# nico-bohlinger/RL-X

Measured on AMD Instinct MI355X. Metric: env-steps/sec (whole node) PPO 4096 envs at 1/2/4/8 MI355X, higher is better.
Workload: dtype f32

## Files before the change

rl-x_amd/csrc/common.h:

```cpp
#pragma once
#include <hip/hip_runtime.h>
#include <hip/hip_ext.h>
#include <stdint.h>
#include <cstring>
#include <cmath>
#include <string>
#include <vector>
#include <functional>
#include "../../include/rlx_hip.h"

namespace rlx {

void set_error(const std::string& msg);

#define RLX_HIP_TRY(expr)                                                                      \
  do {                                                                                         \
    hipError_t e_ = (expr);                                                                    \
    if (e_ != hipSuccess) {                                                                    \
      ::rlx::set_error(std::string(#expr) + " failed: " + hipGetErrorString(e_) + " (" __FILE__ \
                       ":" + std::to_string(__LINE__) + ")");                                  \
      return RLX_EHIP;                                                                         \
    }                                                                                          \
  } while (0)

#define RLX_REQUIRE(cond, code, msg)                 \
  do {                                               \
    if (!(cond)) {                                   \
      ::rlx::set_error(std::string(msg));            \
      return (code);                                 \
    }                                                \
  } while (0)

#define RLX_LAUNCH_CHECK()                           \
  RLX_HIP_TRY(hipGetLastError())

constexpr int WAVE = 64;

struct Scratch {
  void* ptr = nullptr;
  size_t bytes = 0;
};

enum ScratchSlot {
  SL_SORT_KEYS_A = 0, SL_SORT_KEYS_B, SL_SORT_VALS_B, SL_SORT_TMP, SL_PERM,
  SL_MB_X, SL_MB_XC, SL_MB_AUX, SL_STATS,
  SL_ACT_P0, SL_ACT_P1, SL_ACT_P2, SL_ACT_C0, SL_ACT_C1, SL_ACT_C2,
  SL_DACT_0, SL_DACT_1, SL_LN_P, SL_LN_C,
  SL_PARTIAL, SL_HEAD_PART, SL_NORM, SL_NORM2, SL_FWD_A, SL_FWD_B, SL_KEYS, SL_GRAD_P, SL_GRAD_C, SL_MEAN, SL_VALUE, SL_RO_NETS, SL_SAC, SL_LSTM, SL_LSTM_IDX, SL_STAGE, SL_OPT_A, SL_OPT_B, SL_STATS_ALL, SL_ZEROS, SL_STAT_PART, SL_LIDX, SL_COUNTS, SL_DIST_STATS, SL_OVERFLOW, SL_SCHED, SL_NV_ROWS, SL_WFRAG, SL_WFRAG_RO, SL_XMAX, SL_MB_GROUP_X, SL_MB_GROUP_AUX, SL_DZ0, SL_WFRAG_SAC, SL_ROW_REC,
  SL_COUNT
};

enum ProfKernel { PK_GEMM_FWD = 0, PK_GEMM_DX, PK_GEMM_DW, PK_DX_L1BWD,
                  PK_L1FWD, PK_HEAD_LOSS, PK_REDUCE,
                  PK_L12FWD,
                  PK_TAIL,
                  PK_FWD2H,
                  PK_COUNT };
constexpr int PROF_ENGINE_HBM = 2;
struct ProfRec {
  int kid, row;
  double flops, bytes;
  hipEvent_t e0, e1;
};
struct ProfRow {
  int kid, engine;
  int64_t M;
  int N, K;
  int64_t launches, timed;
  double ms, flops, bytes;
};
struct Twin { const void* p[4] = {nullptr, nullptr, nullptr, nullptr}; };

}

struct AttrOnce {
  uint64_t mask = 0;
  static int dev() { int d = 0; (void)hipGetDevice(&d); return d & 63; }
  bool done() const { return (mask >> dev()) & 1; }
  void mark() { mask |= 1ull << dev(); }
};

struct rlx_ctx {
  int device = 0;
  rlx::Scratch slots[3][rlx::SL_COUNT];
  int bank = 0;
  int opt_flip = 0;
  hipStream_t side = nullptr;
  hipEvent_t ev_fork = nullptr, ev_join = nullptr;
  hipEvent_t ev_rows[2] = {nullptr, nullptr};
  hipEvent_t ev_cdone[2] = {nullptr, nullptr};
  const float* dbg_sac_eps[2] = {nullptr, nullptr};
  bool l1fwd_mfma = true;
  bool pipeline_updates = true;
  bool pf_valid = false;
  uint32_t pf_key_in[2] = {0, 0}, pf_key_out[2] = {0, 0};
  int pf_E = 0, pf_scheme = 0;
  int64_t pf_B = 0;
  hipEvent_t pf_done = nullptr;
  hipEvent_t ev_perm_free = nullptr;
  bool perm_free_recorded = false;
  bool two_streams = true;
  const uint32_t* l1_xmax = nullptr;
  const uint32_t* xmax_slot[2] = {nullptr, nullptr};
  int lf_idle_cus = 0;
  bool dw_recompute = false;
  float* l12_stats = nullptr;
  bool l12_ran = false;
  int l1_stats_handover = 1;
  int l1_wrap_refill = 1;
  int64_t dx_l1bwd_wrap_launches = 0;
  int l12_prefetch = 1;
  int64_t l12fwd_pf_launches = 0;
  float* l1_hand_req = nullptr;
  const float* l1_hand[2] = {nullptr, nullptr};
  bool dw_merge = true;
  void* dbg_stamps = nullptr;
  bool fwd2h = true;
  int gather_group_rows = 524288;
  bool gather_records = true;
  bool l12_fused = true;
  int ppo_tail = -1;
  int tail32_waves = 8;
  int ln_row_once = 1;
  int ppo_twin = -1;
  bool fused_recurrent_act = true;
  int num_cus = 256;
  void* defer = nullptr;
  bool prof_on = false;
  int prof_sample = 1;
  hipEvent_t prof_ref = nullptr;
  double prof_union_ms = 0.0;
  std::vector<rlx::ProfRec> prof_recs;
  std::vector<rlx::ProfRow> prof_rows;
  std::vector<hipEvent_t> prof_pool;
  bool gemm_bx = true;
  float bx_gscale = 1.f;
  bool adam_emit = true;
  bool bx_keep[3] = {false, false, false};
  struct RoImages { bool valid = false; const float* params[2] = {nullptr, nullptr}; const void* img[2][3] = {}; int nt[2][3] = {}; } ro_img;
  int bx_force_mi = 0;
  int bx_debug = 0;
  struct BxImage { const float* W; int trans, K, N; const void* img; };
  BxImage bx_img[3][32];
  int bx_n[3] = {0, 0, 0};
  bool disable_l1fused = false;
  std::vector<char> ro_nets_shadow;
  int rank = 0, world = 1;
  void* comm = nullptr;
  hipStream_t comm_stream = nullptr;
  hipEvent_t comm_ev[32] = {};
  int comm_ev_pos = 0;
  rlx_allreduce_fn ar_hook = nullptr;
  void* ar_hook_user = nullptr;
  int ro_exit = 0;
  int64_t bx_window_fallbacks = 0;
  int64_t ar_calls = 0;
  hipStream_t sac_st[2] = {nullptr, nullptr};
  hipEvent_t sac_ev[6] = {nullptr, nullptr, nullptr, nullptr, nullptr, nullptr};
  struct SacImages {
    bool valid = false; const float *pp = nullptr, *qp = nullptr, *qt = nullptr; rlx_mlp_desc pd{}, qd{}; int64_t np = 0, nq2 = 0;
    void written(const float* p, int64_t n) {
      if (!valid) return;
      auto hit = [&](const float* b, int64_t m) { return b && p < b + m && b < p + n; };
      if (hit(pp, np) || hit(qp, nq2) || hit(qt, nq2)) valid = false;
    }
  } sac_img;
  const void* sac_img_arena = nullptr;
  int sac_twin = 1;
  float* sched_host[4] = {nullptr, nullptr, nullptr, nullptr};
  hipEvent_t sched_ev[4] = {nullptr, nullptr, nullptr, nullptr};
  size_t sched_cap = 0;
  int sched_pos = 0;
  int espo_chunk = 2;
  int32_t* espo_host = nullptr;
  hipEvent_t espo_ev[3] = {nullptr, nullptr, nullptr};
  bool pf_dist = false;
  int pf_T = 0, pf_nl = 0, pf_ng = 0, pf_off = 0, pf_mb = 0;
};

namespace rlx {

struct ProfScope {
  rlx_ctx* ctx;
  hipStream_t st;
  int idx = -1;
  ProfScope(rlx_ctx* c, int kid, double flops, hipStream_t s, double bytes = 0.0, int64_t M = 0, int N = 0, int K = 0,
            int engine = 0);
  hipEvent_t ev0() const;
  hipEvent_t ev1() const;
};
#define RLX_PLAUNCH(KERNEL, GRID, BLOCK, LDS, ST, ...)                                                              \
  do {                                                                                                            \
    if (prof.idx >= 0) hipExtLaunchKernelGGL(KERNEL, GRID, BLOCK, LDS, ST, prof.ev0(), prof.ev1(), 0, __VA_ARGS__); \
    else hipLaunchKernelGGL(KERNEL, GRID, BLOCK, LDS, ST, __VA_ARGS__);                                           \
  } while (0)

inline double gemm_bytes(double M, double N, double K, int c_rw = 0) { return 4.0 * (M * K + K * N + M * N * (1 + c_rw)); }

const float* zeros_f32(rlx_ctx* ctx, size_t n);
int ctx_side_stream(rlx_ctx* ctx);
int ctx_sac_streams(rlx_ctx* ctx);
__host__ __device__ __forceinline__ float x_pow2_inv(float m) {
  union { float f; uint32_t u; } c;
  c.f = m;
  const int e = (int)((c.u >> 23) & 0xffu);
  if (e == 0 || e == 0xff) return 1.f;
  int se = 254 - e;
// ... 298 lines not shown
```

rl-x_amd/csrc/core.hip:

```cpp
#include "common.h"
#include <algorithm>
#include <cstdio>
#include <cstdlib>
#include <utility>

namespace rlx {

static thread_local std::string g_last_error;

void set_error(const std::string& msg) { g_last_error = msg; }

void* scratch(rlx_ctx* ctx, ScratchSlot s, size_t bytes) {
  Scratch& sl = ctx->slots[ctx->bank][s];
  if (sl.bytes >= bytes && sl.ptr) return sl.ptr;
  if (sl.ptr) {
    if (hipDeviceSynchronize() != hipSuccess) { set_error("hipDeviceSynchronize failed in scratch()"); return nullptr; }
    (void)hipFree(sl.ptr);
    sl.ptr = nullptr;
    sl.bytes = 0;
  }
  size_t want = ((bytes > (size_t(1) << 20) ? bytes + bytes / 8 : bytes) + 255) & ~size_t(255);
  void* p = nullptr;
  hipError_t e = hipMalloc(&p, want);
  if (e != hipSuccess) {
// ... 145 lines not shown
      flops_out[r.kid] += r.flops;
      bytes_out[r.kid] += r.bytes;
      count_out[r.kid] += 1;
      rlx::ProfRow& q = ctx->prof_rows[r.row];
      q.timed += 1;
      q.ms += ms;
      q.flops += r.flops;
      q.bytes += r.bytes;
      if (q.engine != rlx::PROF_ENGINE_HBM && ctx->prof_ref && hipEventElapsedTime(&t0, ctx->prof_ref, r.e0) == hipSuccess)
        iv.emplace_back(t0, t0 + ms);
    }
    ctx->prof_pool.push_back(r.e0);
    ctx->prof_pool.push_back(r.e1);
  }
  ctx->prof_recs.clear();
  std::sort(iv.begin(), iv.end());
  double uni = 0.0;
  float cs = 0.f, ce = -1.f;
  for (auto& p : iv) {
    if (ce < 0.f || p.first > ce) { if (ce >= 0.f) uni += ce - cs; cs = p.first; ce = p.second; }
    else if (p.second > ce) ce = p.second;
  }
  if (ce >= 0.f) uni += ce - cs;
  ctx->prof_union_ms = uni;
  return RLX_OK;
}

int rlx_prof_rows(rlx_ctx* ctx, rlx_prof_row* rows, int capacity, int* n_out) {
  RLX_REQUIRE(ctx && n_out && (rows || capacity == 0), RLX_EINVAL, "rlx_prof_rows: NULL pointer");
  const int n = (int)ctx->prof_rows.size();
  *n_out = n;
  for (int i = 0; i < n && i < capacity; ++i) {
    const rlx::ProfRow& q = ctx->prof_rows[i];
    rows[i] = rlx_prof_row{q.kid, q.engine, q.N, q.K, q.M, q.launches, q.timed, q.ms, q.flops, q.bytes};
  }
  return RLX_OK;
}

int rlx_prof_union_ms(rlx_ctx* ctx, double* out) {
  RLX_REQUIRE(ctx && out, RLX_EINVAL, "rlx_prof_union_ms: NULL pointer");
  *out = ctx->prof_union_ms;
  return RLX_OK;
}

int rlx_dbg_set_option(rlx_ctx* ctx, const char* name, int value) {
  RLX_REQUIRE(ctx && name, RLX_EINVAL, "rlx_dbg_set_option: NULL");
  if (std::string(name) == "sac_twin") { ctx->sac_twin = value; return RLX_OK; }
  if (std::string(name) == "disable_l1fused") { ctx->disable_l1fused = value != 0; return RLX_OK; }
  if (std::string(name) == "l1fwd_mfma") { ctx->l1fwd_mfma = value != 0; return RLX_OK; }
  if (std::string(name) == "pipeline_updates") { ctx->pipeline_updates = value != 0; return RLX_OK; }
  if (std::string(name) == "two_streams") { ctx->two_streams = value != 0; return RLX_OK; }
  if (std::string(name) == "ppo_twin") { ctx->ppo_twin = value; return RLX_OK; }
  if (std::string(name) == "ro_exit") { ctx->ro_exit = value; return RLX_OK; }
  if (std::string(name) == "lf_idle_cus") { ctx->lf_idle_cus = value < 0 ? 0 : value; return RLX_OK; }
  if (std::string(name) == "dw_recompute") { ctx->dw_recompute = value != 0; return RLX_OK; }
  if (std::string(name) == "dw_merge") { ctx->dw_merge = value != 0; return RLX_OK; }
  if (std::string(name) == "fwd2h") { ctx->fwd2h = value != 0; return RLX_OK; }
  if (std::string(name) == "l12_fused") { ctx->l12_fused = value != 0; return RLX_OK; }
  if (std::string(name) == "gather_group_rows") { ctx->gather_group_rows = value; return RLX_OK; }
  if (std::string(name) == "gather_records") { ctx->gather_records = value != 0; return RLX_OK; }
  if (std::string(name) == "ppo_tail") { ctx->ppo_tail = value < 0 ? -1 : (value > 2 ? 2 : value); return RLX_OK; }
  if (std::string(name) == "tail32_waves") {
    RLX_REQUIRE(value == 4 || value == 8, RLX_EINVAL, "rlx_dbg_set_option: tail32_waves is 4 or 8");
    ctx->tail32_waves = value;
    return RLX_OK;
  }
  if (std::string(name) == "ln_row_once") {
    RLX_REQUIRE(value == 0 || value == 1, RLX_EINVAL, "rlx_dbg_set_option: ln_row_once is 0 or 1");
    ctx->ln_row_once = value;
    return RLX_OK;
  }
  if (std::string(name) == "l1_stats_handover") {
    RLX_REQUIRE(value == 0 || value == 1, RLX_EINVAL, "rlx_dbg_set_option: l1_stats_handover is 0 or 1");
    ctx->l1_stats_handover = value;
    return RLX_OK;
  }
  if (std::string(name) == "l1_wrap_refill") {
    RLX_REQUIRE(value == 0 || value == 1, RLX_EINVAL, "rlx_dbg_set_option: l1_wrap_refill is 0 or 1");
    ctx->l1_wrap_refill = value;
    return RLX_OK;
  }
  if (std::string(name) == "l12_prefetch") {
    RLX_REQUIRE(value == 0 || value == 1, RLX_EINVAL, "rlx_dbg_set_option: l12_prefetch is 0 or 1");
    ctx->l12_prefetch = value;
    return RLX_OK;
  }
  if (std::string(name) == "bx_force_mi") { ctx->bx_force_mi = value; return RLX_OK; }
  if (std::string(name) == "adam_emit") { ctx->adam_emit = value != 0; return RLX_OK; }
  if (std::string(name) == "bx_debug") { ctx->bx_debug = value; return RLX_OK; }
  if (std::string(name) == "bx_gscale_log2") { ctx->bx_gscale = ldexpf(1.f, value < 0 ? 0 : (value > 40 ? 40 : value)); return RLX_OK; }
  if (std::string(name) == "gemm_bx") { ctx->gemm_bx = value != 0; return RLX_OK; }
  if (std::string(name) == "prof_sample") { ctx->prof_sample = value < 1 ? 1 : value; return RLX_OK; }
  if (std::string(name) == "espo_chunk") { ctx->espo_chunk = value < 1 ? 1 : value; return RLX_OK; }
  if (std::string(name) == "fused_recurrent_act") { ctx->fused_recurrent_act = value != 0; return RLX_OK; }
  RLX_REQUIRE(false, RLX_EINVAL, "rlx_dbg_set_option: unknown option");
}

int rlx_dbg_get_counter(rlx_ctx* ctx, const char* name, int64_t* out) {
  RLX_REQUIRE(ctx && name && out, RLX_EINVAL, "rlx_dbg_get_counter: NULL");
  int bank = 0, slot = 0;
  if (sscanf(name, "scratch_ptr:%d:%d", &bank, &slot) == 2 && bank >= 0 && bank < 3 && slot >= 0 && slot < rlx::SL_COUNT) {
    *out = (int64_t)reinterpret_cast<uintptr_t>(ctx->slots[bank][slot].ptr);
    return RLX_OK;
  }
  if (sscanf(name, "scratch_bytes:%d:%d", &bank, &slot) == 2 && bank >= 0 && bank < 3 && slot >= 0 && slot < rlx::SL_COUNT) {
    *out = (int64_t)ctx->slots[bank][slot].bytes;
    return RLX_OK;
  }
  if (std::string(name) == "allreduce_calls") { *out = ctx->ar_calls; return RLX_OK; }
  if (std::string(name) == "dx_l1bwd_wrap_launches") { *out = ctx->dx_l1bwd_wrap_launches; return RLX_OK; }
  if (std::string(name) == "l12fwd_pf_launches") { *out = ctx->l12fwd_pf_launches; return RLX_OK; }
  if (std::string(name) == "bx_window_fallbacks") { *out = ctx->bx_window_fallbacks; return RLX_OK; }
  if (std::string(name) == "gemm_bx") { *out = ctx->gemm_bx ? 1 : 0; return RLX_OK; }
  RLX_REQUIRE(false, RLX_EINVAL, "rlx_dbg_get_counter: unknown counter");
}

int rlx_version(void) { return 200; }

const char* rlx_last_error(void) { return rlx::g_last_error.c_str(); }

int rlx_ctx_create(int device, rlx_ctx** out) {
  RLX_REQUIRE(out != nullptr, RLX_EINVAL, "rlx_ctx_create: out is NULL");
  int count = 0;
  RLX_HIP_TRY(hipGetDeviceCount(&count));
  RLX_REQUIRE(device >= 0 && device < count, RLX_EINVAL, "rlx_ctx_create: no such HIP device");
  RLX_HIP_TRY(hipSetDevice(device));
  hipDeviceProp_t prop;
  RLX_HIP_TRY(hipGetDeviceProperties(&prop, device));
  rlx_ctx* c = new rlx_ctx();
  c->device = device;
  c->num_cus = prop.multiProcessorCount;
  if (const char* e = getenv("RLX_GEMM_BX")) c->gemm_bx = atoi(e) != 0;
  if (const char* e = getenv("RLX_BX_DEBUG")) c->bx_debug = atoi(e);
  *out = c;
  return RLX_OK;
}

int rlx_dist_release(rlx_ctx* ctx);

int rlx_ctx_destroy(rlx_ctx* ctx) {
  if (!ctx) return RLX_OK;
  (void)hipSetDevice(ctx->device);
  (void)hipDeviceSynchronize();
  (void)rlx_dist_release(ctx);
  for (int i = 0; i < 2; ++i)
    if (ctx->sac_st[i]) (void)hipStreamDestroy(ctx->sac_st[i]);
  for (int i = 0; i < 6; ++i)
    if (ctx->sac_ev[i]) (void)hipEventDestroy(ctx->sac_ev[i]);
  for (int i = 0; i < 4; ++i) {
    if (ctx->sched_host[i]) (void)hipHostFree(ctx->sched_host[i]);
    if (ctx->sched_ev[i]) (void)hipEventDestroy(ctx->sched_ev[i]);
  }
  if (ctx->espo_host) (void)hipHostFree(ctx->espo_host);
  for (int i = 0; i < 3; ++i)
    if (ctx->espo_ev[i]) (void)hipEventDestroy(ctx->espo_ev[i]);
  for (int b = 0; b < 3; ++b)
    for (int i = 0; i < rlx::SL_COUNT; ++i)
      if (ctx->slots[b][i].ptr) (void)hipFree(ctx->slots[b][i].ptr);
  if (ctx->ev_fork) (void)hipEventDestroy(ctx->ev_fork);
  if (ctx->ev_join) (void)hipEventDestroy(ctx->ev_join);
  for (int p = 0; p < 2; ++p) {
    if (ctx->ev_rows[p]) (void)hipEventDestroy(ctx->ev_rows[p]);
    if (ctx->ev_cdone[p]) (void)hipEventDestroy(ctx->ev_cdone[p]);
  }
// ... 17 lines not shown
```

rl-x_amd/csrc/rollout.hip:

```cpp
#include "env_device.h"
#include "gemm.h"
#include "mlp.h"
#include "gemm_bx.h"
#include "ppo_internal.h"

namespace rlx {

constexpr int RO_ROWS = 32;
constexpr int RO_THREADS = 256;
constexpr int RO_MAXH = 512;
constexpr int RO_MAXN = 256;
constexpr int RO_A0 = RO_ROWS * (RO_MAXH + 1);
constexpr int RO_A1 = RO_ROWS * (RO_MAXN + 1);
constexpr int RO_BS = G_BK * (RO_MAXN + 4);
constexpr int RO_MISC = 1024 + 64;
constexpr int RO_LDS_FLOATS = RO_A0 + RO_A1 + RO_BS + RO_MISC;
constexpr float RO_LOG_2PI = 1.8378770664093453f;

#define RO_ACT_SWITCH(ACTV, ...)                                                                                      \
  if ((ACTV) == RLX_ACT_ELU) { auto actf = [](float v_) { return act_fwd_t<RLX_ACT_ELU>(v_); }; __VA_ARGS__ }          \
  else if ((ACTV) == RLX_ACT_TANH) { auto actf = [](float v_) { return act_fwd_t<RLX_ACT_TANH>(v_); }; __VA_ARGS__ }   \
  else { const int act_rt_ = (ACTV); auto actf = [act_rt_](float v_) { return act_fwd(v_, act_rt_); }; __VA_ARGS__ }

struct RolloutNet {
// ... 572 lines not shown
          a.env.final_obs[o] = ox[q];
          if (2 * p + 1 < O) a.env.final_obs[o + 1] = oy[q];
        }
      }
    }
  }
  __syncthreads();
  RO_STAMP(8)
  if (t < RO_ROWS) {
    const int64_t n = r0 + t;
    int done = 0;
    if (n < a.N) {
      float lp = 0.f;
      for (int j = 0; j < A; ++j) lp += s_lp[t * A + j];
      a.logp[n] = lp;
      if (a.env.enabled) {
        float acc = 0.f;
        for (int j = 0; j < A; ++j) acc += s_cost[t * A + j];
        const EnvLaneOut e = env_lane_finish_v(a.env.seed, (uint32_t)(n + a.env.env_id_offset), a.env.t, A, a.env.horizon,
                                               a.env.p_term, a.env.reward_noise, acc, es_in, er_in, a.env.ep_step, a.env.ep_ret,
                                               a.env.last_ret, a.env.last_len, (int)n);
        done = e.done;
        a.env.reward[n] = e.reward;
        a.env.terminated[n] = e.term ? 1.f : 0.f;
        if (a.env.episode_stats && e.done) {
          atomicAdd(&a.env.episode_stats[0], 1.f);
          atomicAdd(&a.env.episode_stats[1], e.fin_ret);
          atomicAdd(&a.env.episode_stats[2], e.fin_len);
        }
      }
    }
    s_done[t] = done;
  }
  if (!a.env.enabled) return;
  __syncthreads();
  RO_STAMP(9)
#pragma unroll
  for (int q = 0; q < OPI; ++q) {
    const int it = t + q * RO_THREADS;
    if (it >= RO_ROWS * pairs) continue;
    const int e = it / pairs, p = it - e * pairs;
    const int64_t n = r0 + e;
    if (n >= a.N) continue;
    float x = ox[q], y = oy[q];
    if (s_done[e]) obs_pair(a.env.seed, (uint32_t)(n + a.env.env_id_offset), a.env.t, ENV_STREAM_RESET + p, x, y);
    const int64_t o = n * O + 2 * p;
    a.obs_out[o] = x;
    if (2 * p + 1 < O) a.obs_out[o + 1] = y;
  }
  RO_STAMP(10)
#undef RO_STAMP
}

static bool fill_net(const rlx_mlp_desc& d, const float* params, RolloutNet* n) {
  const MlpLayout L = make_layout(d);
  n->params = params;
  n->n_hidden = d.n_hidden;
  n->out_dim = d.out_dim;
  n->act = d.act;
  n->ln_first = d.ln_first;
  if (d.n_hidden < 1 || d.n_hidden > 3 || d.in_dim < 1 || d.in_dim > 32 || d.out_dim < 1) return false;
  if (d.hidden[0] < 64 || d.hidden[0] % 64 != 0 || d.hidden[0] > RO_MAXH) return false;
  for (int l = 0; l < d.n_hidden; ++l) {
    n->hidden[l] = d.hidden[l];
    n->W[l] = L.layer[l].W;
    n->b[l] = L.layer[l].b;
    if (l >= 1 && d.hidden[l] != 128 && d.hidden[l] != 256) return false;
    if (l >= 1 && d.hidden[l - 1] % (2 * G_BK) != 0) return false;
  }
  n->g0 = L.layer[0].g;
  n->be0 = L.layer[0].be;
  n->headW = L.head.W;
  n->headb = L.head.b;
  n->logstd = L.logstd;
  return d.out_dim * RO_ROWS <= 1024;
}

static int upload_nets_and_launch(rlx_ctx* ctx, const RolloutNet (&hn)[2], RolloutArgs& a, hipStream_t st) {
  RolloutNet* dn = (RolloutNet*)scratch(ctx, SL_RO_NETS, sizeof(hn));
  if (!dn) return RLX_ENOMEM;
  if (ctx->ro_nets_shadow.size() != sizeof(hn) || memcmp(ctx->ro_nets_shadow.data(), hn, sizeof(hn)) != 0) {
    RLX_HIP_TRY(hipStreamSynchronize(st));
    RLX_HIP_TRY(hipMemcpy(dn, hn, sizeof(hn), hipMemcpyHostToDevice));
    ctx->ro_nets_shadow.assign(reinterpret_cast<const char*>(hn), reinterpret_cast<const char*>(hn) + sizeof(hn));
  }
  a.nets = dn;
  static AttrOnce attr_set;      
  const size_t lds = (size_t)RO_LDS_FLOATS * sizeof(float);
  if (!attr_set.done()) {
    RLX_HIP_TRY(hipFuncSetAttribute(reinterpret_cast<const void*>(k_rollout_step),
                                    hipFuncAttributeMaxDynamicSharedMemorySize, (int)lds));
    attr_set.mark();  
  }
  const int grid = div_up(a.N, RO_ROWS) * 2;
  hipLaunchKernelGGL(k_rollout_step, dim3(grid), dim3(RO_THREADS), lds, st, a);
  RLX_LAUNCH_CHECK();
  return RLX_OK;
}

bool rollout_decoder_supported(const RolloutDecoder& p, const rlx_mlp_desc& cd) {
  RolloutNet c;
  return p.K0 % 64 == 0 && p.K0 >= 64 && p.K0 <= RO_MAXN && p.hidden[0] % 256 == 0 && p.hidden[0] <= RO_MAXH &&
         (p.hidden[1] == 128 || p.hidden[1] == 256) && (p.hidden[2] == 128 || p.hidden[2] == 256) &&
         p.out_dim * RO_ROWS <= 1024 && fill_net(cd, nullptr, &c) && cd.out_dim == 1;
}

int launch_rollout_decoder(rlx_ctx* ctx, const RolloutDecoder& p, const rlx_mlp_desc& cd, const float* cparams,
                           const float* obs, int O, uint32_t k0, uint32_t k1, int scheme, float* action, float* processed,
                           float* value, float* logp, int N, int clip_and_rescale, const float* lo, const float* hi,
                           int noise_row_offset, int N_global, int deterministic, hipStream_t st) {
  RLX_REQUIRE(rollout_decoder_supported(p, cd), RLX_EUNSUP, "rollout decoder: shape outside the fused kernel's envelope");
  RolloutNet hn[2];
  memset(hn, 0, sizeof(hn));
  RolloutNet& n = hn[0];
  n.params = p.params; n.n_hidden = 3; n.out_dim = p.out_dim; n.act = p.act; n.ln_first = 1;
  for (int l = 0; l < 3; ++l) { n.hidden[l] = p.hidden[l]; n.W[l] = p.W[l]; n.b[l] = p.b[l]; }
  n.g0 = p.g0; n.be0 = p.be0; n.headW = p.headW; n.headb = p.headb; n.logstd = p.logstd;
  n.wide_in = p.K0; n.x_wide = p.x; n.x_b = p.xb; n.xb_dim = p.xb ? 64 : 0; n.xb_g = p.xb_g; n.xb_be = p.xb_be;
  fill_net(cd, cparams, &hn[1]);
  if (ctx->ro_img.valid && ctx->gemm_bx && ctx->ro_img.params[0] == p.params && ctx->ro_img.params[1] == cparams) {
    for (int q = 0; q < 2; ++q)
      for (int l = 1; l < 3; ++l) { hn[q].img[l] = ctx->ro_img.img[q][l]; hn[q].img_nt[l] = ctx->ro_img.nt[q][l]; }
  }
  RolloutArgs a{};
  a.obs_in = obs; a.obs_out = nullptr; a.action = action; a.processed = processed; a.value = value; a.logp = logp;
  a.N = N; a.O = O; a.A = p.out_dim;
  a.k0 = k0; a.k1 = k1; a.scheme = scheme;
  a.clip_and_rescale = clip_and_rescale; a.lo = lo; a.hi = hi;
  a.noise_row_offset = noise_row_offset; a.N_global = N_global; a.deterministic = deterministic;
  a.env.enabled = 0;
  return upload_nets_and_launch(ctx, hn, a, st);
}

}

using namespace rlx;

extern "C" {

int rlx_ppo_rollout_step_supported(const rlx_mlp_desc* pdesc, const rlx_mlp_desc* cdesc) {
  if (!pdesc || !cdesc) return 0;
  RolloutNet a, b;
  return (fill_net(*pdesc, nullptr, &a) && fill_net(*cdesc, nullptr, &b) && pdesc->in_dim == cdesc->in_dim &&
          pdesc->has_logstd && cdesc->out_dim == 1)
             ? 1 : 0;
}

int rlx_ppo_rollout_begin(rlx_ctx* ctx, const rlx_mlp_desc* pdesc, const float* pparams, const rlx_mlp_desc* cdesc,
                          const float* cparams, void* stream) {
// ... 67 lines not shown
                             const float* act_low, const float* act_high, int noise_row_offset, int N_global,
                             int fuse_env, uint32_t env_seed, int env_id_offset, uint32_t env_t, int horizon,
                             float p_term, float reward_noise, float* final_obs, float* reward, float* terminated,
                             int32_t* ep_step, float* ep_ret, float* last_ret, float* last_len, float* episode_stats,
                             void* stream) {
  RLX_REQUIRE(ctx && pdesc && pparams && cdesc && cparams && obs_in && key_io && action && value && logp, RLX_EINVAL,
              "rlx_ppo_rollout_step_f32: NULL pointer");
  RLX_REQUIRE(N > 0 && N_global >= N, RLX_EINVAL, "rlx_ppo_rollout_step_f32: bad sizes");
  RLX_REQUIRE(rlx_ppo_rollout_step_supported(pdesc, cdesc), RLX_EUNSUP,
              "rlx_ppo_rollout_step_f32: network shape outside the fused kernel's envelope "
              "(use rlx_actor_critic_fwd_sample_f32 + rlx_env_step_f32)");
  RLX_REQUIRE(!clip_and_rescale || (act_low && act_high), RLX_EINVAL, "rlx_ppo_rollout_step_f32: clip needs bounds");
  if (fuse_env)
    RLX_REQUIRE(obs_out && final_obs && reward && terminated && ep_step && ep_ret && last_ret && last_len && horizon > 0,
                RLX_EINVAL, "rlx_ppo_rollout_step_f32: fuse_env needs the env state pointers");
  RolloutArgs a{};
  RolloutNet hn[2];
  memset(hn, 0, sizeof(hn));
  fill_net(*pdesc, pparams, &hn[0]);
  fill_net(*cdesc, cparams, &hn[1]);
  if (ctx->ro_img.valid && ctx->gemm_bx && ctx->ro_img.params[0] == pparams && ctx->ro_img.params[1] == cparams) {
    for (int n = 0; n < 2; ++n)
      for (int l = 1; l < 3; ++l) { hn[n].img[l] = ctx->ro_img.img[n][l]; hn[n].img_nt[l] = ctx->ro_img.nt[n][l]; }
  }
  a.obs_in = obs_in; a.obs_out = obs_out; a.action = action; a.processed = processed; a.value = value; a.logp = logp;
  a.N = N; a.O = pdesc->in_dim; a.A = pdesc->out_dim;
  uint32_t ks[4];
  split_host(key_io, ks, 2, scheme);
  key_io[0] = ks[0]; key_io[1] = ks[1];
  a.k0 = ks[2]; a.k1 = ks[3]; a.scheme = scheme;
  a.clip_and_rescale = clip_and_rescale; a.lo = act_low; a.hi = act_high;
  a.noise_row_offset = noise_row_offset; a.N_global = N_global;
  a.dbg_exit = ctx->ro_exit;
  a.stamps = (unsigned long long*)ctx->dbg_stamps;
  a.env.enabled = fuse_env ? 1 : 0;
  a.env.seed = env_seed; a.env.env_id_offset = env_id_offset; a.env.t = env_t; a.env.horizon = horizon;
  a.env.p_term = p_term; a.env.reward_noise = reward_noise; a.env.final_obs = final_obs; a.env.reward = reward;
  a.env.terminated = terminated; a.env.ep_step = ep_step; a.env.ep_ret = ep_ret; a.env.last_ret = last_ret;
  a.env.last_len = last_len; a.env.episode_stats = episode_stats;
  return upload_nets_and_launch(ctx, hn, a, (hipStream_t)stream);
}

int rlx_ppo_rollout_f32(rlx_ctx* ctx, const rlx_mlp_desc* pdesc, const float* pparams, const rlx_mlp_desc* cdesc,
                        const float* cparams, float* states, float* obs_last, uint32_t key_io[2], int scheme, float* actions,
                        float* values, float* logps, int T, int N, int clip_and_rescale, const float* act_low,
                        const float* act_high, int noise_row_offset, int N_global, uint32_t env_seed, int env_id_offset,
                        uint32_t env_t0, int horizon, float p_term, float reward_noise, float* final_obs, float* rewards,
                        float* terminated, int32_t* ep_step, float* ep_ret, float* last_ret, float* last_len,
                        float* episode_stats, void* stream) {
  RLX_REQUIRE(ctx && pdesc && states && obs_last && actions && values && logps && final_obs && rewards && terminated, RLX_EINVAL,
              "rlx_ppo_rollout_f32: NULL pointer");
  RLX_REQUIRE(T > 0 && N > 0, RLX_EINVAL, "rlx_ppo_rollout_f32: bad sizes");
  const int64_t O = pdesc->in_dim, A = pdesc->out_dim;
  for (int t = 0; t < T; ++t) {
    const int rc = rlx_ppo_rollout_step_f32(
        ctx, pdesc, pparams, cdesc, cparams, states + (int64_t)t * N * O, t + 1 < T ? states + (int64_t)(t + 1) * N * O : obs_last,
        key_io, scheme, actions + (int64_t)t * N * A, nullptr, values + (int64_t)t * N, logps + (int64_t)t * N, N, clip_and_rescale,
        act_low, act_high, noise_row_offset, N_global, 1, env_seed, env_id_offset, env_t0 + (uint32_t)t, horizon, p_term,
        reward_noise, final_obs + (int64_t)t * N * O, rewards + (int64_t)t * N, terminated + (int64_t)t * N, ep_step, ep_ret,
        last_ret, last_len, episode_stats, stream);
    if (rc) return rc;
  }
  return RLX_OK;
}

}
```

Before: 8.348 million.

## Add persistent multi-step rollout kernel that runs chunks of env steps per launch

Adds k_rollout_steps, which runs up to 32 rollout steps inside one launch instead of one kernel launch per step. Observations stay in LDS between steps with double buffering, and episode counters stay in registers. Noise and observation draws for the next step are overlapped with the env-finish work on other waves. This is meant to remove per-step launch overhead and the global round-trips for obs and weights, at the cost of higher register and LDS use, a separate critic episode-step buffer, and a large new code path that must reproduce the old semantics exactly.

Result: faster. 8.442 million (median of 6 runs) (+1.1%).

```diff
diff --git a/rl-x_amd/csrc/common.h b/rl-x_amd/csrc/common.h
--- a/rl-x_amd/csrc/common.h
+++ b/rl-x_amd/csrc/common.h
@@ -46,7 +46,7 @@
   SL_MB_X, SL_MB_XC, SL_MB_AUX, SL_STATS,
   SL_ACT_P0, SL_ACT_P1, SL_ACT_P2, SL_ACT_C0, SL_ACT_C1, SL_ACT_C2,
   SL_DACT_0, SL_DACT_1, SL_LN_P, SL_LN_C,
-  SL_PARTIAL, SL_HEAD_PART, SL_NORM, SL_NORM2, SL_FWD_A, SL_FWD_B, SL_KEYS, SL_GRAD_P, SL_GRAD_C, SL_MEAN, SL_VALUE, SL_RO_NETS, SL_SAC, SL_LSTM, SL_LSTM_IDX, SL_STAGE, SL_OPT_A, SL_OPT_B, SL_STATS_ALL, SL_ZEROS, SL_STAT_PART, SL_LIDX, SL_COUNTS, SL_DIST_STATS, SL_OVERFLOW, SL_SCHED, SL_NV_ROWS, SL_WFRAG, SL_WFRAG_RO, SL_XMAX, SL_MB_GROUP_X, SL_MB_GROUP_AUX, SL_DZ0, SL_WFRAG_SAC, SL_ROW_REC,
+  SL_PARTIAL, SL_HEAD_PART, SL_NORM, SL_NORM2, SL_FWD_A, SL_FWD_B, SL_KEYS, SL_GRAD_P, SL_GRAD_C, SL_MEAN, SL_VALUE, SL_RO_NETS, SL_SAC, SL_LSTM, SL_LSTM_IDX, SL_STAGE, SL_OPT_A, SL_OPT_B, SL_STATS_ALL, SL_ZEROS, SL_STAT_PART, SL_LIDX, SL_COUNTS, SL_DIST_STATS, SL_OVERFLOW, SL_SCHED, SL_NV_ROWS, SL_WFRAG, SL_WFRAG_RO, SL_XMAX, SL_MB_GROUP_X, SL_MB_GROUP_AUX, SL_DZ0, SL_WFRAG_SAC, SL_ROW_REC, SL_RO_CRITIC_ES,
   SL_COUNT
 };
 
@@ -153,6 +153,11 @@
   rlx_allreduce_fn ar_hook = nullptr;
   void* ar_hook_user = nullptr;
   int ro_exit = 0;
+  int ro_persistent = 1;
+  int ro_chunk_steps = 32;
+  int64_t ro_persistent_launches = 0;
+  int64_t ro_step_launches = 0;
+  const void* ro_critic_es = nullptr;
   int64_t bx_window_fallbacks = 0;
   int64_t ar_calls = 0;
   hipStream_t sac_st[2] = {nullptr, nullptr};
diff --git a/rl-x_amd/csrc/core.hip b/rl-x_amd/csrc/core.hip
--- a/rl-x_amd/csrc/core.hip
+++ b/rl-x_amd/csrc/core.hip
@@ -221,6 +221,16 @@
   if (std::string(name) == "two_streams") { ctx->two_streams = value != 0; return RLX_OK; }
   if (std::string(name) == "ppo_twin") { ctx->ppo_twin = value; return RLX_OK; }
   if (std::string(name) == "ro_exit") { ctx->ro_exit = value; return RLX_OK; }
+  if (std::string(name) == "rollout_persistent") {
+    RLX_REQUIRE(value == 0 || value == 1, RLX_EINVAL, "rlx_dbg_set_option: rollout_persistent is 0 or 1");
+    ctx->ro_persistent = value;
+    return RLX_OK;
+  }
+  if (std::string(name) == "rollout_chunk_steps") {
+    RLX_REQUIRE(value >= 1 && value <= 64, RLX_EINVAL, "rlx_dbg_set_option: rollout_chunk_steps is 1 .. 64");
+    ctx->ro_chunk_steps = value;
+    return RLX_OK;
+  }
   if (std::string(name) == "lf_idle_cus") { ctx->lf_idle_cus = value < 0 ? 0 : value; return RLX_OK; }
   if (std::string(name) == "dw_recompute") { ctx->dw_recompute = value != 0; return RLX_OK; }
   if (std::string(name) == "dw_merge") { ctx->dw_merge = value != 0; return RLX_OK; }
@@ -279,6 +289,9 @@
   if (std::string(name) == "allreduce_calls") { *out = ctx->ar_calls; return RLX_OK; }
   if (std::string(name) == "dx_l1bwd_wrap_launches") { *out = ctx->dx_l1bwd_wrap_launches; return RLX_OK; }
   if (std::string(name) == "l12fwd_pf_launches") { *out = ctx->l12fwd_pf_launches; return RLX_OK; }
+  if (std::string(name) == "ro_persistent_launches") { *out = ctx->ro_persistent_launches; return RLX_OK; }
+  if (std::string(name) == "ro_step_launches") { *out = ctx->ro_step_launches; return RLX_OK; }
+  if (std::string(name) == "ro_critic_es_ptr") { *out = (int64_t)reinterpret_cast<uintptr_t>(ctx->ro_critic_es); return RLX_OK; }
   if (std::string(name) == "bx_window_fallbacks") { *out = ctx->bx_window_fallbacks; return RLX_OK; }
   if (std::string(name) == "gemm_bx") { *out = ctx->gemm_bx ? 1 : 0; return RLX_OK; }
   RLX_REQUIRE(false, RLX_EINVAL, "rlx_dbg_get_counter: unknown counter");
diff --git a/rl-x_amd/csrc/rollout.hip b/rl-x_amd/csrc/rollout.hip
--- a/rl-x_amd/csrc/rollout.hip
+++ b/rl-x_amd/csrc/rollout.hip
@@ -648,6 +648,383 @@
 #undef RO_STAMP
 }
 
+constexpr int RO_MAX_CHUNK = 64;
+struct RolloutStepsLayout { int a1, wh, outs, lp, xs, eps, ox, red, done, keys, cst, total; };
+struct RolloutStepsArgs {
+  RolloutArgs a;
+  int S;
+  int last_chunk;
+  float* obs_last;
+  int32_t* critic_es;
+  RolloutStepsLayout L;
+  uint32_t keys[2 * RO_MAX_CHUNK];
+};
+
+__global__ __launch_bounds__(RO_THREADS, 2) void k_rollout_steps(RolloutStepsArgs g) {
+  extern __shared__ __attribute__((aligned(16))) float smem[];
+  const RolloutArgs& a = g.a;
+  float* A0 = smem;
+  float* A1 = smem + g.L.a1;
+  float* Whs = smem + g.L.wh;
+  float* outs = smem + g.L.outs;
+  float* s_lp = smem + g.L.lp;
+  float* Xs0 = smem + g.L.xs;
+  float* eps_s = smem + g.L.eps;
+  float* ox_s = smem + g.L.ox;
+  float* red0 = smem + g.L.red;
+  int* s_done = reinterpret_cast<int*>(smem + g.L.done);
+  uint32_t* keys_s = reinterpret_cast<uint32_t*>(smem + g.L.keys);
+  float* ls_s = smem + g.L.cst;
+  float *sd_s = ls_s + 32, *lo_s = ls_s + 64, *hi_s = ls_s + 96, *hb_s = ls_s + 128;
+  const int t = threadIdx.x, lane = t & 63, w = t >> 6;
+  const int which = blockIdx.x & 1;
+  const int64_t r0 = (int64_t)(blockIdx.x >> 1) * RO_ROWS;
+  const RolloutNet* __restrict__ np = a.nets + which;
+  typedef const float __attribute__((address_space(1))) * gf32_t;
+  const float* P = np->params;
+  gf32_t Pg = (gf32_t)P;
+  const int n_hidden = np->n_hidden, act = np->act, ln_first = np->ln_first, OD = np->out_dim;
+  const int H1 = np->hidden[1], H2 = np->hidden[2];
+  const int64_t oW0 = np->W[0], ob0 = np->b[0], ob1 = np->b[1], ob2 = np->b[2];
+  const int64_t og0 = np->g0, obe0 = np->be0, oHW = np->headW, oHb = np->headb;
+  const int64_t oLS = a.nets[0].logstd;
+  const u32x4* img1 = reinterpret_cast<const u32x4*>(np->img[1]);
+  const u32x4* img2 = reinterpret_cast<const u32x4*>(np->img[2]);
+  const int imgnt1 = np->img_nt[1], imgnt2 = np->img_nt[2];
+  const int O = a.O, A = a.A, S = g.S;
+  const int pairs = (O + 1) / 2;
+  float* oy_s = ox_s + RO_ROWS * pairs;
+  float* s_cost = s_lp + RO_ROWS * A;
+  const int64_t NO = (int64_t)a.N * O, NA = (int64_t)a.N * A;
+  constexpr int H0 = 512, NT0 = 4, NW0 = RO_THREADS / 64, KS0 = 16, st = H0 + 1;
+  constexpr int EPI = (RO_ROWS * 32 + RO_THREADS - 1) / RO_THREADS;
+  constexpr int OPI = (RO_ROWS * 16 + RO_THREADS - 1) / RO_THREADS;
+  const int OP = (O + 1) & ~1;
+  const int li = lane & 31, lh = lane >> 5;
+  const bool lb0 = (lane & 1) != 0, lb1 = (lane & 2) != 0;
+  const int colbase = w * 32 * NT0 + li;
+  const int hk = n_hidden > 2 ? H2 : H1;
+
+  {
+    uint32_t kv = 0;
+#pragma unroll
+    for (int i = 0; i < 2 * RO_MAX_CHUNK; ++i) kv = (t == i) ? g.keys[i] : kv;
+    if (t < 2 * RO_MAX_CHUNK) keys_s[t] = kv;
+  }
+  float w0r[KS0][NT0];
+#define RO_LOAD_W0                                                                                                  \
+  {                                                                                                                 \
+    int zw_;                                                                                                        \
+    asm volatile("s_mov_b32 %0, 0" : "=s"(zw_));                                                                    \
+    gf32_t w0a_ = Pg + oW0 + (int)(threadIdx.x >> 6) * 32 * NT0 + (int)(threadIdx.x & 31) + zw_;                    \
+    gf32_t w0b_ = w0a_ + (int)((threadIdx.x >> 5) & 1) * 512;                                                       \
+    const bool lo_half_ = ((threadIdx.x >> 5) & 1) == 0;                                                            \
+    _Pragma("unroll") for (int s_ = 0; s_ < KS0; ++s_) {                                                            \
+      if (2 * s_ + 1 < O) {                                                                                         \
+        _Pragma("unroll") for (int j = 0; j < NT0; ++j) w0r[s_][j] = w0b_[(2 * s_) * 512 + 32 * j];                 \
+      } else if (2 * s_ < O) {                                                                                      \
+        _Pragma("unroll") for (int j = 0; j < NT0; ++j) {                                                           \
+          const float v_ = w0a_[(2 * s_) * 512 + 32 * j];                                                           \
+          w0r[s_][j] = lo_half_ ? v_ : 0.f;                                                                         \
+        }                                                                                                           \
+      } else {                                                                                                      \
+        _Pragma("unroll") for (int j = 0; j < NT0; ++j) w0r[s_][j] = 0.f;                                           \
+      }                                                                                                             \
+    }                                                                                                               \
+  }
+  RO_LOAD_W0
+  float b0v[NT0], gam[NT0], bet[NT0];
+#pragma unroll
+  for (int j = 0; j < NT0; ++j) {
+    b0v[j] = Pg[ob0 + colbase + 32 * j];
+    gam[j] = ln_first ? Pg[og0 + colbase + 32 * j] : 1.f;
+    bet[j] = ln_first ? Pg[obe0 + colbase + 32 * j] : 0.f;
+  }
+  if (t < 32) {
+    hb_s[t] = t < OD ? Pg[oHb + t] : 0.f;
+    const bool in = which == 0 && t < A;
+    const float ls = in ? Pg[oLS + t] : 0.f;
+    ls_s[t] = ls;
+    sd_s[t] = expf(ls);
+    lo_s[t] = in && a.clip_and_rescale ? a.lo[t] : 0.f;
+    hi_s[t] = in && a.clip_and_rescale ? a.hi[t] : 0.f;
+  }
+  for (int i = t; i < hk * OD; i += RO_THREADS) Whs[i] = Pg[oHW + i];
+  int es_r = 0;
+  float er_r = 0.f;
+  if (t < RO_ROWS && r0 + t < a.N) {
+    if (which == 0) { es_r = a.env.ep_step[r0 + t]; er_r = a.env.ep_ret[r0 + t]; }
+    else es_r = g.critic_es[r0 + t];
+  }
+  for (int i = t; i < 2 * RO_ROWS * 33; i += RO_THREADS) Xs0[i] = 0.f;
+  __syncthreads();
+  {
+    constexpr int XPI = RO_ROWS * 32 / RO_THREADS;
+#pragma unroll
+    for (int c = 0; c < XPI; ++c) {
+      const int i = t + c * RO_THREADS, r = i >> 5, k = i & 31;
+      if (k < O && r0 + r < a.N) Xs0[r * 33 + k] = a.obs_in[(r0 + r) * O + k];
+    }
+  }
+  auto draw_step = [&](int tid, int nthr, bool noise, uint32_t k0, uint32_t k1, uint32_t tt) {
+    if (noise) {
+      const uint64_t total = (uint64_t)a.N_global * A;
+      for (int it = tid; it < RO_ROWS * A; it += nthr) {
+        const int e = it / A, j = it - e * A;
+        const int64_t n = r0 + e;
+        float v = 0.f;
+        if (n < a.N) v = normal_from_bits(random_bits_at(k0, k1, (uint64_t)(n + a.noise_row_offset) * A + j, total, a.scheme));
+        eps_s[it] = v;
+      }
+    }
+    for (int it = tid; it < RO_ROWS * pairs; it += nthr) {
+      const int e = it / pairs, p = it - e * pairs;
+      const int64_t n = r0 + e;
+      float x = 0.f, y = 0.f;
+      if (n < a.N) obs_pair(a.env.seed, (uint32_t)(n + a.env.env_id_offset), tt, (uint32_t)p, x, y);
+      ox_s[it] = x;
+      oy_s[it] = y;
+    }
+  };
+  if (which == 0) draw_step(t, RO_THREADS, true, g.keys[0], g.keys[1], a.env.t);
+  __syncthreads();
+
+  int cur = 0;
+  const int t_launch = t;
+  for (int s = 0; s < S; ++s) {
+    int tv;
+    asm volatile("v_mov_b32 %0, %1" : "=v"(tv) : "v"(t_launch));
+    const int t = tv, lane = t & 63, w = t >> 6;
+    const int li = lane & 31, lh = lane >> 5;
+    const bool lb0 = (lane & 1) != 0, lb1 = (lane & 2) != 0;
+    const int colbase = w * 32 * NT0 + li;
+    const float* Xc = Xs0 + cur * (RO_ROWS * 33);
+    float* Xn = Xs0 + (cur ^ 1) * (RO_ROWS * 33);
+    const uint32_t tt = a.env.t + (uint32_t)s;
+    f32x16 z[NT0];
+#pragma unroll
+    for (int j = 0; j < NT0; ++j) {
+#pragma unroll
+      for (int r = 0; r < 16; ++r) z[j][r] = b0v[j];
+    }
+    {
+      const float* x0 = Xc + li * 33 + lh;
+#pragma unroll
+      for (int s_ = 0; s_ < KS0; ++s_) {
+        if (2 * s_ < OP) {
+          const float av = x0[2 * s_];
+#pragma unroll
+          for (int j = 0; j < NT0; ++j) z[j] = __builtin_amdgcn_mfma_f32_32x32x2f32(av, w0r[s_][j], z[j], 0, 0, 0);
+        }
+      }
+    }
+    float* tot0 = red0 + 2 * NW0 * 32 + w * 64;
+    if (ln_first) {
+#pragma unroll
+      for (int gq = 0; gq < 4; ++gq) {
+        float sv[4], ssv[4];
+#pragma unroll
+        for (int e = 0; e < 4; ++e) {
+          float s_ = 0.f, ss = 0.f;
+#pragma unroll
+          for (int j = 0; j < NT0; ++j) { s_ += z[j][4 * gq + e]; ss += z[j][4 * gq + e] * z[j][4 * gq + e]; }
+          sv[e] = s_;
+          ssv[e] = ss;
+        }
+        const float st_ = half_sum4(sv[0], sv[1], sv[2], sv[3], lb0, lb1);
+        const float sst = half_sum4(ssv[0], ssv[1], ssv[2], ssv[3], lb0, lb1);
+        if (li < 4) {
+          red0[(0 * NW0 + w) * 32 + 8 * gq + 4 * lh + li] = st_;
+          red0[(1 * NW0 + w) * 32 + 8 * gq + 4 * lh + li] = sst;
+        }
+      }
+      __syncthreads();
+      float v = 0.f;
+#pragma unroll
+      for (int q = 0; q < NW0; ++q) v += red0[((lane >> 5) * NW0 + q) * 32 + (lane & 31)];
+      tot0[lane] = v;
+    }
+    const float invH = 1.0f / (float)H0;
+    if (ln_first) {
+      RO_ACT_SWITCH(act,
+        _Pragma("unroll") for (int gq = 0; gq < 4; ++gq) {
+          _Pragma("unroll") for (int e = 0; e < 4; ++e) {
+            const int r = 4 * gq + e, row = 8 * gq + 4 * lh + e;
+            const float mean = tot0[row] * invH;
+            const float rs = rsqrtf(fmaxf(0.f, tot0[32 + row] * invH - mean * mean) + 1e-6f);
+            _Pragma("unroll") for (int j = 0; j < NT0; ++j)
+              A0[row * st + colbase + 32 * j] = actf((z[j][r] - mean) * rs * gam[j] + bet[j]);
+          }
+        })
+    } else {
+      RO_ACT_SWITCH(act,
+        _Pragma("unroll") for (int gq = 0; gq < 4; ++gq) {
+          _Pragma("unroll") for (int e = 0; e < 4; ++e) {
+            const int r = 4 * gq + e, row = 8 * gq + 4 * lh + e;
+            _Pragma("unroll") for (int j = 0; j < NT0; ++j) A0[row * st + colbase + 32 * j] = actf(z[j][r]);
+          }
+        })
+    }
+    if (H1 == 256) fused_layer_bx<2>(A0, H0 + 1, H0, img1, imgnt1, P + ob1, A1, H1 + 1, act, t);
+    else fused_layer_bx<1>(A0, H0 + 1, H0, img1, imgnt1, P + ob1, A1, H1 + 1, act, t);
+    const float* hin = A1;
+    int hst = H1 + 1;
+    if (n_hidden > 2) {
+      if (H2 == 256) fused_layer_bx<2>(A1, H1 + 1, H1, img2, imgnt2, P + ob2, A0, H2 + 1, act, t);
+      else fused_layer_bx<1>(A1, H1 + 1, H1, img2, imgnt2, P + ob2, A0, H2 + 1, act, t);
+      hin = A0; hst = H2 + 1;
+    }
+    {
+      const int r = t & 31;
+      const float* hr = hin + r * hst;
+#pragma unroll
+      for (int i = 0; i < 4; ++i) {
+        const int o = (t >> 5) + 8 * i;
+        if (o < OD) {
+          float acc0 = 0.f, acc1 = 0.f;
+#pragma unroll 4
+          for (int k = 0; k < hk; k += 2) {
+            acc0 = fmaf(hr[k], Whs[k * OD + o], acc0);
+            acc1 = fmaf(hr[k + 1], Whs[(k + 1) * OD + o], acc1);
+          }
+          outs[r * OD + o] = (acc0 + acc1) + hb_s[o];
+        }
+      }
+    }
+    __syncthreads();
+    RO_LOAD_W0
+    int te;
+    asm volatile("v_mov_b32 %0, %1" : "=v"(te) : "v"(t_launch));
+    {
+    const int t = te, w = t >> 6;
+    if (which == 1) {
+      if (t < RO_ROWS && r0 + t < a.N) a.value[(int64_t)s * a.N + r0 + t] = outs[t];
+      if (w == 0) {
+        if (t < RO_ROWS) {
+          const int64_t n = r0 + t;
+          int done = 0;
+          if (n < a.N) {
+            uint32_t x0 = tt, x1 = ENV_STREAM_MISC;
+            threefry2x32(a.env.seed, (uint32_t)(n + a.env.env_id_offset), x0, x1);
+            const float ut = bits_to_unit(x1);
+            const int es = es_r + 1;
+            done = (ut < a.env.p_term || es >= a.env.horizon) ? 1 : 0;
+            es_r = done ? 0 : es;
+          }
+          s_done[t] = done;
+        }
+      } else if (s + 1 < S) draw_step(t - 64, RO_THREADS - 64, false, 0u, 0u, tt);
+      if (s + 1 == S) break;
+      __syncthreads();
+      for (int it = t; it < RO_ROWS * pairs; it += RO_THREADS) {
+        const int e = it / pairs, p = it - e * pairs;
+        const int64_t n = r0 + e;
+        if (n >= a.N) continue;
+        float x = ox_s[it], y = oy_s[it];
+        if (s_done[e]) obs_pair(a.env.seed, (uint32_t)(n + a.env.env_id_offset), tt, ENV_STREAM_RESET + p, x, y);
+        Xn[e * 33 + 2 * p] = x;
+        if (2 * p + 1 < O) Xn[e * 33 + 2 * p + 1] = y;
+      }
+      cur ^= 1;
+      __syncthreads();
+      continue;
+    }
+    float* action_t = a.action + (int64_t)s * NA;
+    float* final_t = a.env.final_obs + (int64_t)s * NO;
+    float* obs_out = (g.last_chunk && s + 1 == S) ? g.obs_last : a.obs_out + (int64_t)s * NO;
+#pragma unroll
+    for (int q = 0; q < EPI; ++q) {
+      const int it = t + q * RO_THREADS;
+      if (it >= RO_ROWS * A) continue;
+      const int e = it / A, j = it - e * A;
+      const int64_t n = r0 + e;
+      if (n >= a.N) continue;
+      const float eps = eps_s[it];
+      const float ls = ls_s[j];
+      const float sd = sd_s[j];
+      const float mu = outs[it];
+      const float act = mu + sd * eps;
+      const float zs = (act - mu) / sd;
+      s_lp[it] = -0.5f * zs * zs - 0.5f * RO_LOG_2PI - ls;
+      action_t[n * A + j] = act;
+      float p = act;
+      if (a.clip_and_rescale) {
+        const float c = fminf(fmaxf(act, -1.f), 1.f);
+        p = lo_s[j] + 0.5f * (c + 1.0f) * (hi_s[j] - lo_s[j]);
+      }
+      const float d = env_cost_diff(p, Xc[e * 33 + j % O]);
+      s_cost[it] = d * d;
+    }
+    float ox[OPI], oy[OPI];
+#pragma unroll
+    for (int q = 0; q < OPI; ++q) {
+      const int it = t + q * RO_THREADS;
+      ox[q] = oy[q] = 0.f;
+      if (it < RO_ROWS * pairs) {
+        const int e = it / pairs, p = it - e * pairs;
+        const int64_t n = r0 + e;
+        ox[q] = ox_s[it];
+        oy[q] = oy_s[it];
+        if (n < a.N) {
+          const int64_t o = n * O + 2 * p;
+          final_t[o] = ox[q];
+          if (2 * p + 1 < O) final_t[o + 1] = oy[q];
+        }
+      }
+    }
+    __syncthreads();
+    if (w == 0) {
+      if (t < RO_ROWS) {
+        const int64_t n = r0 + t;
+        int done = 0;
+        if (n < a.N) {
+          float lp = 0.f;
+          for (int j = 0; j < A; ++j) lp += s_lp[t * A + j];
+          a.logp[(int64_t)s * a.N + n] = lp;
+          float acc = 0.f;
+          for (int j = 0; j < A; ++j) acc += s_cost[t * A + j];
+          const EnvLaneOut e = env_lane_finish_v(a.env.seed, (uint32_t)(n + a.env.env_id_offset), tt, A, a.env.horizon, a.env.p_term,
+                                                 a.env.reward_noise, acc, es_r, er_r, a.env.ep_step, a.env.ep_ret, a.env.last_ret,
+                                                 a.env.last_len, (int)n);
+          done = e.done;
+          er_r = e.done ? 0.f : er_r + e.reward;
+          es_r = e.done ? 0 : es_r + 1;
+          a.env.reward[(int64_t)s * a.N + n] = e.reward;
+          a.env.terminated[(int64_t)s * a.N + n] = e.term ? 1.f : 0.f;
+          if (a.env.episode_stats && e.done) {
+            atomicAdd(&a.env.episode_stats[0], 1.f);
+            atomicAdd(&a.env.episode_stats[1], e.fin_ret);
+            atomicAdd(&a.env.episode_stats[2], e.fin_len);
+          }
+        }
+        s_done[t] = done;
+      }
+    } else if (s + 1 < S) {
+      draw_step(t - 64, RO_THREADS - 64, true, keys_s[2 * s + 2], keys_s[2 * s + 3], tt + 1u);
+    }
+    __syncthreads();
+#pragma unroll
+    for (int q = 0; q < OPI; ++q) {
+      const int it = t + q * RO_THREADS;
+      if (it >= RO_ROWS * pairs) continue;
+      const int e = it / pairs, p = it - e * pairs;
+      const int64_t n = r0 + e;
+      if (n >= a.N) continue;
+      float x = ox[q], y = oy[q];
+      if (s_done[e]) obs_pair(a.env.seed, (uint32_t)(n + a.env.env_id_offset), tt, ENV_STREAM_RESET + p, x, y);
+      const int64_t o = n * O + 2 * p;
+      obs_out[o] = x;
+      Xn[e * 33 + 2 * p] = x;
+      if (2 * p + 1 < O) { obs_out[o + 1] = y; Xn[e * 33 + 2 * p + 1] = y; }
+    }
+    cur ^= 1;
+    __syncthreads();
+    }
+  }
+  if (which == 1 && t < RO_ROWS && r0 + t < a.N) g.critic_es[r0 + t] = es_r;
+#undef RO_LOAD_W0
+}
+
 static bool fill_net(const rlx_mlp_desc& d, const float* params, RolloutNet* n) {
   const MlpLayout L = make_layout(d);
   n->params = params;
@@ -672,7 +1049,37 @@
   return d.out_dim * RO_ROWS <= 1024;
 }
 
-static int upload_nets_and_launch(rlx_ctx* ctx, const RolloutNet (&hn)[2], RolloutArgs& a, hipStream_t st) {
+constexpr int RO_STEPS_MAX_LDS = 160 * 1024;
+static bool ro_steps_layout(const RolloutNet (&hn)[2], int O, int A, RolloutStepsLayout* L) {
+  int h1 = 0, wh = 0, od = 0;
+  for (int n = 0; n < 2; ++n) {
+    const RolloutNet& q = hn[n];
+    if (q.wide_in != 0 || q.hidden[0] != 512 || O > 32 || q.n_hidden < 2 || q.n_hidden > 3) return false;
+    for (int l = 1; l < q.n_hidden; ++l)
+      if (!q.img[l]) return false;
+    const int hk = q.hidden[q.n_hidden - 1];
+    h1 = q.hidden[1] > h1 ? q.hidden[1] : h1;
+    wh = hk * q.out_dim > wh ? hk * q.out_dim : wh;
+    od = q.out_dim > od ? q.out_dim : od;
+  }
+  auto up4 = [](int x) { return (x + 3) & ~3; };
+  const int pairs = (O + 1) / 2;
+  L->a1 = RO_ROWS * (512 + 1);
+  L->wh = L->a1 + up4(RO_ROWS * (h1 + 1));
+  L->outs = L->wh + up4(wh);
+  L->lp = L->outs + up4(RO_ROWS * od);
+  L->xs = L->lp + up4(2 * RO_ROWS * A);
+  L->eps = L->xs + up4(2 * RO_ROWS * 33);
+  L->ox = L->eps + up4(RO_ROWS * A);
+  L->red = L->ox + up4(2 * RO_ROWS * pairs);
+  L->done = L->red + 2 * 4 * 32 + 4 * 64;
+  L->keys = L->done + RO_ROWS;
+  L->cst = L->keys + 2 * RO_MAX_CHUNK;
+  L->total = L->cst + 5 * 32;
+  return (size_t)L->total * sizeof(float) <= (size_t)RO_STEPS_MAX_LDS;
+}
+
+static int upload_nets(rlx_ctx* ctx, const RolloutNet (&hn)[2], RolloutArgs& a, hipStream_t st) {
   RolloutNet* dn = (RolloutNet*)scratch(ctx, SL_RO_NETS, sizeof(hn));
   if (!dn) return RLX_ENOMEM;
   if (ctx->ro_nets_shadow.size() != sizeof(hn) || memcmp(ctx->ro_nets_shadow.data(), hn, sizeof(hn)) != 0) {
@@ -681,7 +1088,13 @@
     ctx->ro_nets_shadow.assign(reinterpret_cast<const char*>(hn), reinterpret_cast<const char*>(hn) + sizeof(hn));
   }
   a.nets = dn;
-  static AttrOnce attr_set;      
+  return RLX_OK;
+}
+
+static int upload_nets_and_launch(rlx_ctx* ctx, const RolloutNet (&hn)[2], RolloutArgs& a, hipStream_t st) {
+  const int rc = upload_nets(ctx, hn, a, st);
+  if (rc) return rc;
+  static AttrOnce attr_set;
   const size_t lds = (size_t)RO_LDS_FLOATS * sizeof(float);
   if (!attr_set.done()) {
     RLX_HIP_TRY(hipFuncSetAttribute(reinterpret_cast<const void*>(k_rollout_step),
@@ -691,6 +1104,7 @@
   const int grid = div_up(a.N, RO_ROWS) * 2;
   hipLaunchKernelGGL(k_rollout_step, dim3(grid), dim3(RO_THREADS), lds, st, a);
   RLX_LAUNCH_CHECK();
+  ++ctx->ro_step_launches;
   return RLX_OK;
 }
 
@@ -864,6 +1278,70 @@
               "rlx_ppo_rollout_f32: NULL pointer");
   RLX_REQUIRE(T > 0 && N > 0, RLX_EINVAL, "rlx_ppo_rollout_f32: bad sizes");
   const int64_t O = pdesc->in_dim, A = pdesc->out_dim;
+  if (ctx->ro_persistent && ctx->ro_exit == 0 && !ctx->dbg_stamps && pparams && cdesc && cparams && key_io && N_global >= N &&
+      rlx_ppo_rollout_step_supported(pdesc, cdesc) && (!clip_and_rescale || (act_low && act_high)) && ep_step && ep_ret &&
+      last_ret && last_len && horizon > 0 && ctx->ro_img.valid && ctx->gemm_bx && ctx->ro_img.params[0] == pparams &&
+      ctx->ro_img.params[1] == cparams) {
+    RolloutNet hn[2];
+    memset(hn, 0, sizeof(hn));
+    fill_net(*pdesc, pparams, &hn[0]);
+    fill_net(*cdesc, cparams, &hn[1]);
+    for (int n = 0; n < 2; ++n)
+      for (int l = 1; l < 3; ++l) { hn[n].img[l] = ctx->ro_img.img[n][l]; hn[n].img_nt[l] = ctx->ro_img.nt[n][l]; }
+    RolloutStepsLayout L;
+    if (ro_steps_layout(hn, (int)O, (int)A, &L)) {
+      RolloutStepsArgs g{};
+      RolloutArgs& a = g.a;
+      a.N = N; a.O = (int)O; a.A = (int)A; a.scheme = scheme;
+      a.clip_and_rescale = clip_and_rescale; a.lo = act_low; a.hi = act_high;
+      a.noise_row_offset = noise_row_offset; a.N_global = N_global;
+      a.env.enabled = 1;
+      a.env.seed = env_seed; a.env.env_id_offset = env_id_offset; a.env.horizon = horizon;
+      a.env.p_term = p_term; a.env.reward_noise = reward_noise; a.env.ep_step = ep_step; a.env.ep_ret = ep_ret;
+      a.env.last_ret = last_ret; a.env.last_len = last_len; a.env.episode_stats = episode_stats;
+      g.obs_last = obs_last;
+      g.L = L;
+      g.critic_es = (int32_t*)scratch(ctx, SL_RO_CRITIC_ES, (size_t)N * sizeof(int32_t));
+      if (!g.critic_es) return RLX_ENOMEM;
+      ctx->ro_critic_es = g.critic_es;
+      hipStream_t st = (hipStream_t)stream;
+      const int rc = upload_nets(ctx, hn, a, st);
+      if (rc) return rc;
+      RLX_HIP_TRY(hipMemcpyAsync(g.critic_es, ep_step, (size_t)N * sizeof(int32_t), hipMemcpyDeviceToDevice, st));
+      static AttrOnce attr_set;
+      if (!attr_set.done()) {
+        RLX_HIP_TRY(hipFuncSetAttribute(reinterpret_cast<const void*>(k_rollout_steps), hipFuncAttributeMaxDynamicSharedMemorySize,
+                                        RO_STEPS_MAX_LDS));
+        attr_set.mark();
+      }
+      const int chunk = ctx->ro_chunk_steps < 1 ? 1 : (ctx->ro_chunk_steps > RO_MAX_CHUNK ? RO_MAX_CHUNK : ctx->ro_chunk_steps);
+      const int grid = div_up(N, RO_ROWS) * 2;
+      for (int t0 = 0; t0 < T; t0 += chunk) {
+        const int S = T - t0 < chunk ? T - t0 : chunk;
+        for (int s = 0; s < S; ++s) {
+          uint32_t ks[4];
+          split_host(key_io, ks, 2, scheme);
+          key_io[0] = ks[0]; key_io[1] = ks[1];
+          g.keys[2 * s] = ks[2]; g.keys[2 * s + 1] = ks[3];
+        }
+        g.S = S;
+        g.last_chunk = t0 + S == T ? 1 : 0;
+        a.obs_in = states + (int64_t)t0 * N * O;
+        a.obs_out = states + (int64_t)(t0 + 1) * N * O;
+        a.action = actions + (int64_t)t0 * N * A;
+        a.value = values + (int64_t)t0 * N;
+        a.logp = logps + (int64_t)t0 * N;
+        a.env.t = env_t0 + (uint32_t)t0;
+        a.env.final_obs = final_obs + (int64_t)t0 * N * O;
+        a.env.reward = rewards + (int64_t)t0 * N;
+        a.env.terminated = terminated + (int64_t)t0 * N;
+        hipLaunchKernelGGL(k_rollout_steps, dim3(grid), dim3(RO_THREADS), (size_t)L.total * sizeof(float), st, g);
+        RLX_LAUNCH_CHECK();
+        ++ctx->ro_persistent_launches;
+      }
+      return RLX_OK;
+    }
+  }
   for (int t = 0; t < T; ++t) {
     const int rc = rlx_ppo_rollout_step_f32(
         ctx, pdesc, pparams, cdesc, cparams, states + (int64_t)t * N * O, t + 1 < T ? states + (int64_t)(t + 1) * N * O : obs_last,
```
